# enricobolzonello/TravellingSalesmanOptimization

Measured on AMD Instinct MI355X. Metric: 2-opt delta evals/sec/node (n=4096 EUC_2D, NN(0) tour to 2-opt local optimum), higher is better.
Workload: dtype uint16 costs, int32 deltas

## Files before the change

### include/tspgpu.h

```cpp
#ifndef TSPGPU_H
#define TSPGPU_H

#ifdef __cplusplus
extern "C" {
#endif

typedef struct tspgpu_ctx tspgpu_ctx;

enum { TSPGPU_EUC_2D = 0, TSPGPU_ATT = 1, TSPGPU_CEIL_2D = 2 };

enum { TSPGPU_ELEM_AUTO = 0, TSPGPU_ELEM_F64 = 1, TSPGPU_ELEM_I32 = 2, TSPGPU_ELEM_U16 = 3 };

enum {
    TSPGPU_OPT_ELEM = 1,
    TSPGPU_OPT_KERNEL = 2,
    TSPGPU_OPT_BATCH = 3,
    TSPGPU_OPT_WGS_PER_TOUR = 4,
    TSPGPU_OPT_HISTORY = 5,
    TSPGPU_OPT_GRAPH = 6,
    TSPGPU_OPT_TIMING = 7,
    TSPGPU_OPT_BLOCK = 8,
    TSPGPU_OPT_MAX_TOURS = 9,
    TSPGPU_OPT_DEPTH = 10,
    TSPGPU_OPT_FUSED = 12,
// ... 95 lines not shown
int tspgpu_tour_copy(tspgpu_ctx *ctx, int dst, int src);
int tspgpu_tour_two_opt(tspgpu_ctx *ctx, int slot, long max_sweeps, double time_left_s, long *sweeps);
int tspgpu_tour_or_opt(tspgpu_ctx *ctx, int slot, long max_moves, double time_left_s, long *moves);
int tspgpu_tour_local_search(tspgpu_ctx *ctx, int slot, double time_left_s,
                             long *two_opt_sweeps, long *or_moves, int *rounds);
int tspgpu_tours_local_search(tspgpu_ctx *ctx, int slot0, int count, double time_left_s,
                              long *two_opt_sweeps, long *or_moves, int *rounds);
int tspgpu_time_or_sweep(tspgpu_ctx *ctx, int slot, int reps, float *ms_mean);
int tspgpu_tour_sweep_part(tspgpu_ctx *ctx, int slot, int part, int nparts, double *delta, int *a, int *b);
int tspgpu_tour_apply_move(tspgpu_ctx *ctx, int slot, int a, int b, double delta);
int tspgpu_tour_store(tspgpu_ctx *ctx, int slot, int *path, double *cost, double *last_delta);
int tspgpu_time_sweep(tspgpu_ctx *ctx, int slot, int reps, float *ms_mean);
int tspgpu_time_build(tspgpu_ctx *ctx, int reps, float *ms_mean);
int tspgpu_timing_read(tspgpu_ctx *ctx, double *sweep_ms_total, long *sweep_launches, int reset);
int tspgpu_debug_stamps(tspgpu_ctx *ctx, unsigned long long *out, int capacity_words);
int tspgpu_history(tspgpu_ctx *ctx, int *a, int *b, double *delta, int capacity, int *count);

int tspgpu_two_opt_multi_once(tspgpu_ctx *ctx, int *path, double *cost, int *nmoves,
                              int *moves_ab , double *deltas , int cap);
int tspgpu_two_opt_multi(tspgpu_ctx *ctx, int *path, double *cost, double time_left_s, long *sweeps, long *moves);
int tspgpu_tour_two_opt_multi(tspgpu_ctx *ctx, int slot, long max_sweeps, double time_left_s, long *sweeps, long *moves);
int tspgpu_time_multi_sweep(tspgpu_ctx *ctx, int slot, int reps, float *ms_mean);

int tspgpu_neighbours_build(tspgpu_ctx *ctx, int K);
int tspgpu_neighbours_get(tspgpu_ctx *ctx, int *nodes , double *weights );
int tspgpu_two_opt_nl_once(tspgpu_ctx *ctx, int *path, double *cost, int *nmoves,
                           int *moves_ab , double *deltas , int cap);
int tspgpu_two_opt_nl(tspgpu_ctx *ctx, int *path, double *cost, double time_left_s, int polish,
                      long *sweeps, long *moves, long *polish_sweeps, long *polish_moves);
int tspgpu_tour_two_opt_nl(tspgpu_ctx *ctx, int slot, long max_sweeps, double time_left_s, long *sweeps, long *moves);
// ... 49 lines not shown
```

### travellingsalesmanoptimization_amd/_lib.py

```python
import ctypes as C
import os

import numpy as np

HERE = os.path.dirname(os.path.abspath(__file__))
LIB_PATH = os.path.join(HERE, "csrc", "libtspgpu.so")

T_OK, CANCELLED, UNKNOWN, INVALID_ARGUMENT, DEADLINE_EXCEEDED = 0, 1, 2, 3, 4
RESOURCE_EXHAUSTED, FAILED_PRECONDITION, UNIMPLEMENTED, INTERNAL, UNAVAILABLE = 8, 9, 12, 13, 14

EUC_2D, ATT, CEIL_2D = 0, 1, 2
ELEM_AUTO, ELEM_F64, ELEM_I32, ELEM_U16 = 0, 1, 2, 3
OPT_ELEM, OPT_KERNEL, OPT_BATCH, OPT_WGS_PER_TOUR, OPT_HISTORY = 1, 2, 3, 4, 5
OPT_GRAPH, OPT_TIMING, OPT_BLOCK, OPT_MAX_TOURS, OPT_DEPTH, OPT_MATRIX_FREE, OPT_FUSED, OPT_SWEEP_CAP, OPT_NN_KERNEL, OPT_PIPE2 = 6, 7, 8, 9, 10, 11, 12, 13, 14, 15
OPT_PERSIST, OPT_PERSIST_EDGES, OPT_PERSIST_WINDOW, OPT_BUILD_KERNEL, OPT_STREAM_PERSIST = 16, 17, 18, 19, 20
OPT_EM_FORM = 21
OPT_OR_MATRIX_FREE = 22
INFO_OR_OTF, INFO_OR_OTF_R = 34, 35
INFO_MULTI_SWEEPS, INFO_MULTI_MOVES, INFO_MULTI_MAX_MOVES, INFO_MULTI_R, INFO_MULTI_THREADS, INFO_MULTI_NCH = 36, 37, 38, 39, 40, 41
INFO_NL_K, INFO_NL_SWEEPS, INFO_NL_MOVES, INFO_NL_POLISH_SWEEPS, INFO_NL_NODES = 42, 43, 44, 45, 46
INFO_OR_NL_SWEEPS, INFO_OR_NL_MOVES, INFO_OR_NL_MAX_MOVES, INFO_OR_NL_ROUNDS, INFO_OR_NL_STARTS = 47, 48, 49, 50, 51
INFO_NL_BATCH_TOURS, INFO_NL_BATCH_LAUNCHES, INFO_NL_BATCH_MAX_LIVE, INFO_NL_BATCH_WGS = 52, 53, 54, 55
INFO_VNS_NL_WALKS, INFO_VNS_NL_ITERATIONS, INFO_VNS_NL_ROUNDS, INFO_VNS_NL_MAX_LIVE, INFO_VNS_NL_DRY = 56, 57, 58, 59, 60
INFO_THREE_NL_W, INFO_THREE_NL_SWEEPS, INFO_THREE_NL_MOVES, INFO_THREE_NL_MAX_MOVES, INFO_THREE_NL_PHASES, INFO_THREE_NL_NODES = 62, 63, 64, 65, 66, 67
EM_FORM_AUTO, EM_FORM_RESIDENT, EM_FORM_PER_STEP = 0, 1, 2
MOPT_EXCHANGE = 1000
EXCHANGE_AUTO, EXCHANGE_HOST, EXCHANGE_RCCL = 0, 1, 2

_dp = np.ctypeslib.ndpointer(dtype=np.float64, flags="C_CONTIGUOUS")
_ip = np.ctypeslib.ndpointer(dtype=np.int32, flags="C_CONTIGUOUS")
_pd = C.POINTER(C.c_double)
_pi = C.POINTER(C.c_int)
_pl = C.POINTER(C.c_long)
_ctx = C.c_void_p

SIGNATURES = {
    "tspgpu_device_count": (C.c_int, []),
    "tspgpu_create": (C.c_int, [C.c_int, C.POINTER(_ctx)]),
    "tspgpu_destroy": (None, [_ctx]),
# ... 37 lines not shown
    "tspgpu_multi_prepare": (C.c_int, [_ctx]),
    "tspgpu_multi_set_points": (C.c_int, [_ctx, _dp, C.c_int, C.c_int]),
    "tspgpu_multi_build_costs": (C.c_int, [_ctx]),
    "tspgpu_multi_multistart_nn_2opt": (C.c_int, [_ctx, C.c_void_p, C.c_int, C.c_double, _ip, _pd, _pi, _pl]),
    "tspgpu_multi_multistart_local_search": (C.c_int, [_ctx, C.c_void_p, C.c_int, C.c_double, _ip, _pd, _pi, _pl, _pl]),
    "tspgpu_multi_nn_all": (C.c_int, [_ctx, C.c_void_p, C.c_int, C.c_double, _ip, _pd, _pi, _pi]),
    "tspgpu_tour_load": (C.c_int, [_ctx, C.c_int, _ip]),
    "tspgpu_tour_nn": (C.c_int, [_ctx, C.c_int, C.c_int]),
    "tspgpu_tour_copy": (C.c_int, [_ctx, C.c_int, C.c_int]),
    "tspgpu_tour_two_opt": (C.c_int, [_ctx, C.c_int, C.c_long, C.c_double, _pl]),
    "tspgpu_tour_store": (C.c_int, [_ctx, C.c_int, C.c_void_p, _pd, _pd]),
    "tspgpu_time_sweep": (C.c_int, [_ctx, C.c_int, C.c_int, C.POINTER(C.c_float)]),
    "tspgpu_time_build": (C.c_int, [_ctx, C.c_int, C.POINTER(C.c_float)]),
    "tspgpu_timing_read": (C.c_int, [_ctx, _pd, _pl, C.c_int]),
    "tspgpu_debug_stamps": (C.c_int, [_ctx, C.c_void_p, C.c_int]),
    "tspgpu_history": (C.c_int, [_ctx, _ip, _ip, _dp, C.c_int, _pi]),
    "tspgpu_two_opt_multi_once": (C.c_int, [_ctx, _ip, _pd, _pi, _ip, _dp, C.c_int]),
    "tspgpu_two_opt_multi": (C.c_int, [_ctx, _ip, _pd, C.c_double, _pl, _pl]),
    "tspgpu_tour_two_opt_multi": (C.c_int, [_ctx, C.c_int, C.c_long, C.c_double, _pl, _pl]),
    "tspgpu_time_multi_sweep": (C.c_int, [_ctx, C.c_int, C.c_int, C.POINTER(C.c_float)]),
    "tspgpu_neighbours_build": (C.c_int, [_ctx, C.c_int]),
    "tspgpu_neighbours_get": (C.c_int, [_ctx, _ip, C.c_void_p]),
    "tspgpu_two_opt_nl_once": (C.c_int, [_ctx, _ip, _pd, _pi, _ip, _dp, C.c_int]),
    "tspgpu_two_opt_nl": (C.c_int, [_ctx, _ip, _pd, C.c_double, C.c_int, _pl, _pl, _pl, _pl]),
    "tspgpu_tour_two_opt_nl": (C.c_int, [_ctx, C.c_int, C.c_long, C.c_double, _pl, _pl]),
    "tspgpu_time_nl_sweep": (C.c_int, [_ctx, C.c_int, C.c_int, C.POINTER(C.c_float)]),
    "tspgpu_or_opt_nl_once": (C.c_int, [_ctx, _ip, _pd, _pi, _ip, _dp, C.c_int]),
    "tspgpu_or_opt_nl": (C.c_int, [_ctx, _ip, _pd, C.c_double, _pl, _pl]),
    "tspgpu_tour_or_opt_nl": (C.c_int, [_ctx, C.c_int, C.c_long, C.c_double, _pl, _pl]),
    "tspgpu_local_search_nl": (C.c_int, [_ctx, _ip, _pd, C.c_double, _pl, _pl, _pl, _pl, _pi]),
# ... 34 lines not shown
```

### travellingsalesmanoptimization_amd/csrc/tspgpu.hip

```cpp

#include <hip/hip_runtime.h>
#include <cstddef>

#include <algorithm>
#include <chrono>
#include <cfloat>
#include <climits>
#include <cstdarg>
#include <cstdint>
#include <cstdio>
#include <cstdlib>
#include <cstring>
#include <cmath>
#include <string>
#include <type_traits>
#include <vector>

#include "tspgpu.h"
#include "tspgpu_relaunch.h"

#ifndef TSPGPU_RPC
#define TSPGPU_RPC 3
#endif

enum { E_OK = 0, E_INVALID = 3, E_DEADLINE = 4, E_EXHAUSTED = 8, E_PRECOND = 9,
       E_UNIMPL = 12, E_INTERNAL = 13, E_UNAVAILABLE = 14 };

#define TWO_OPT_EPS (-1.0E-7)

typedef unsigned long long u64;

static constexpr u64 KEY_NONE = ~0ull;
static constexpr int MAX_WGS_PER_TOUR = 1024;

// ... 2597 lines not shown
#include "tspgpu_hipmem.h"
using tspmem::Row; using tspmem::Rows;
#define MEM_GROUP __attribute__((visibility("hidden")))

struct MEM_GROUP ContextMem {
    DevBuf<int> d_flags;
    DevBuf<double2> d_pts;
    DevBuf<int2> d_ipts;
    DevBuf<double2> d_spts;
    PinBuf<int> h_ord;
    DevBuf<double> d_trace;
    HistBuf hist{nullptr, nullptr, nullptr, 0};
    DevBuf<int> hist_a, hist_b; DevBuf<double> hist_d;
    DevBuf<unsigned long long> d_stamps;
    DevBuf<u64> d_lp_slots; PinBuf<int> h_lp;
    DevBuf<int> d_lp_best;
    DevBuf<int> d_vns_rand;
    DevBuf<OrCtl> d_or;
    DevBuf<M2Ctl> d_m2;
};

struct MEM_GROUP InstanceMem {
    M2Buf m2{};
    M2Buf nlb{};
    NlbCtl *d_nlb_ctl = nullptr;
    int nlb_cap = 0;
    int *d_nlv_ord = nullptr, *d_nlv_best = nullptr;
    NlvCtl *d_nlv_ctl = nullptr;
    int nlv_cap = 0;
    DevBuf<int> d_nlv_rand; DevBuf<double> d_nlv_trace;
// ... 114 lines not shown
    int vns_mode = 0;
    long opt_lp_hello = 200000;
    int opt_lp_poll_sleep = 0;
    int opt_vns_launch_k = 65536;
    int opt_lp_fail_at = 0;
    int vns_launch_nrand = 0;
    relaunch::Gate lp_gate;
    bool lp_used = false;
    int opt_stream = 1;
    bool sp_used = false;
    int opt_sp_nch = 0;
    int opt_otf_early = 0;
    bool plan_otf_early = false;
    bool lp_shaped = false;
    int opt_lp_generic = 0;
    bool max16k = false;
    bool max8k = false;

    int opt_em_form = 0;
    int em_form = 0;
    long em_stale = 0, em_steps = 0;

    int or_batch_R = 0;
    int opt_or_otf = 0;
    int opt_or_otf_early = 0;
    int or_otf_form = 0;
    int or_otf_R = 0;

    long m2_sweeps = 0, m2_moves = 0, m2_max_k = 0;

// ... 688 lines not shown
    int e = (n + std::min(ctx->cus, 256) - 1) / std::min(ctx->cus, 256);
    if (ctx->opt_persist_edges > e) e = ctx->opt_persist_edges;
    if (e > LW_EMAX) return false;
    const int ws = (e + n / 2 + 23) & ~7;
    if (ws > n || (ws >> 3) - 1 > LW_BT) return false;
    const size_t nl = (size_t)((n + 7) & ~7);
    if ((nl >> 3) > (size_t)LW_BT) return false;
    const size_t fixed = (size_t)(e + 1) * ws * 2 + (nl + 8) * 4 + 512 + (tabu ? (nl + 16) * 2 : 0);
    int ns = 2;
    if (fixed + 2 * nl * 2 > ctx->lds_max) ns = 1;
    if (fixed + (size_t)ns * nl * 2 > ctx->lds_max) return false;
    E = e; W = (n + e - 1) / e; Ws = ws; nstage = ns; lds = fixed + (size_t)ns * nl * 2;
    return W <= ctx->cus && W <= 256;
}

static const void *lp_shaped_fn(int n, int E)
{
    if (n == 4096 && E == 16) return (const void *)k_lds2opt<true, false, false, 4096, 16>;
    if (n == 1024 && E == 4) return (const void *)k_lds2opt<true, false, false, 1024, 4>;
    return nullptr;
}

static_assert((int)relaunch::INTERNAL == (int)E_INTERNAL && (int)relaunch::GO_ON == (int)E_OK, "the driver's codes are the engine's");
static bool resident_wanted(const tspgpu_ctx *ctx) { return ctx->opt_persist == 2 || (ctx->opt_persist == 1 && ctx->opt_kernel == 0 && ctx->opt_fused == 1); }

template <typename ARGS> static int resident_args(tspgpu_ctx *ctx, ARGS &A, int slot, int W, int budget, bool first)
{
    HIP_TRY(hipMemsetAsync(ctx->d_lp_slots, 0, (size_t)2 * W * 64 + 64, ctx->stream));
    memset(&A, 0, sizeof A);
    A.S = ctx->S; A.mat = (const u16 *)ctx->d_mat.p; A.n = ctx->n; A.ld = ctx->ld; A.slot = slot; A.budget = budget;
    A.slots = ctx->d_lp_slots; A.ctl = reinterpret_cast<int *>(ctx->d_lp_slots + (size_t)2 * W * 8); A.hist = ctx->hist;
    A.hello_ticks = ctx->opt_lp_hello;
    if (ctx->opt_lp_fail_at > 0 && !first) { ctx->opt_lp_fail_at--; A.hello_ticks = -5000; }
    A.spin_ticks = 100000000;
// ... 64 lines not shown
    size_t lds = 0;
    bool win = false;
    if (ctx->opt_persist_window == 1 && persist_fits_w(ctx, E, W, lds, Ws, nstage, tabu != nullptr)) win = true;
    else if (!persist_fits(ctx, E, W, lds, tabu != nullptr)) {
        if (ctx->opt_persist_window == 2 || !persist_fits_w(ctx, E, W, lds, Ws, nstage, tabu != nullptr)) return E_OK;
        win = true;
    }
    if (ctx->lp_gate.skip_this()) return E_OK;
    HIP_TRY(ctx->d_lp_slots.reserve(((size_t)2 * LP_BT * 64 + 64) / 8));
    HIP_TRY(ctx->h_lp.reserve(16));
    if (tabu || vns) HIP_TRY(ctx->d_lp_best.reserve((size_t)ctx->ld + 16));
    const int pk = (tabu ? ctx->max8k : ctx->max16k) ? 1 : 0;
    void (*const fns[2][3][2])(PersistArgs) = {
        {{k_lds2opt<false, false>, k_lds2opt<true, false>}, {k_lds2opt<false, true>, k_lds2opt<true, true>}, {k_lds2opt<false, false, true>, k_lds2opt<true, false, true>}},
        {{k_lds2opt_w<false, false>, k_lds2opt_w<true, false>}, {k_lds2opt_w<false, true>, k_lds2opt_w<true, true>}, {k_lds2opt_w<false, false, true>, k_lds2opt_w<true, false, true>}}};
    const void *const sfn = !win && !tabu && !vns && pk && !ctx->opt_lp_generic ? lp_shaped_fn(ctx->n, E) : nullptr;
    const void *const fn = sfn ? sfn : (const void *)fns[win][tabu ? 1 : vns ? 2 : 0][pk];
    if (const int rc = ensure_max_lds(ctx, fn)) return rc;
    const double t_end = deadline_of(time_left_s);
    if (t_end >= 0 && time_left_s <= 0) { if (deadline_hit) *deadline_hit = true; *ran = true; ctx->lp_used = true; ctx->lp_window = win; ctx->lp_shaped = false; return E_OK; }
    if (vns) vns->need_rand = false;
    auto launch = [&](int budget, bool first, int &status, int &sd, auto &&fill, const double *also = nullptr) -> int {
        PersistArgs A;
        int rc = resident_args(ctx, A, slot, W, budget, first);
        A.E = E; A.nl = (ctx->n + 7) & ~7; A.Ws = Ws; A.nstage = nstage;
        if (!rc) rc = fill(A);
        return rc ? rc : launch_resident(ctx, "LDS-resident descent", fn, W, win ? LW_BT : LP_BT, lds, A, first, status, sd, also);
    };
    auto best_cost = [&]() { return reinterpret_cast<double *>(reinterpret_cast<char *>(ctx->d_tabu) + offsetof(TabuState, best_cost)); };
    auto walk_fill = [&](PersistArgs &A, double best0) -> int {
        HIP_TRY(hipMemsetAsync(ctx->d_lp_best + ctx->ld, 0, 8, ctx->stream));
        A.best0 = best0; A.best_ord = ctx->d_lp_best; A.best_dir = ctx->d_lp_best + ctx->ld; A.best_out = best_cost();
        return E_OK;
    };
    auto walk_completed = [&](int status, int sd) -> int {
        hipLaunchKernelGGL(k_lds_best_succ, dim3((ctx->n + 255) / 256), dim3(256), 0, ctx->stream, ctx->d_lp_best, ctx->d_lp_best + ctx->ld, ctx->d_best_succ, ctx->n);
        HIP_TRY(hipGetLastError());
        return descent_completed(ctx, status, sd);
    };
    relaunch::Result r;
// ... 32 lines not shown
            memcpy(&vns->best, ctx->h_lp + 8, 8);
            if (status == LP_ST_NEED_RAND) {
                vns->need_rand = vns->used + ctx->vns_launch_nrand - ctx->h_lp[5] >= vns->nrand;
                return vns->need_rand ? relaunch::STOP : relaunch::GO_ON;
            }
            if (status == LP_ST_VNS_DONE) return vns->it >= vns->k ? relaunch::STOP : relaunch::GO_ON;
            return next;
        };
        r = relaunch::drive(ctx->lp_gate, now_s, t_end, 8e-6, time_left_io,
                            [&](int budget, bool first, int &st, int &sd) { return launch(budget, first, st, sd, fill, best_cost()); }, completed, hand_over);
    } else
        r = relaunch::drive(ctx->lp_gate, now_s, t_end, 8e-6, time_left_io,
                            [&](int budget, bool first, int &st, int &sd) { return launch(budget, first, st, sd, [](PersistArgs &) -> int { return E_OK; }); },
                            [&](int status, int sd) { return descent_completed(ctx, status, sd); }, hand_over);
    if (const int rc = resident_result(ctx, r, deadline_hit, ran); rc || !*ran) return rc;
    ctx->lp_used = true; ctx->lp_window = win; ctx->lp_shaped = sfn != nullptr;
    return E_OK;
}

static bool stream_fits(const tspgpu_ctx *ctx, int &P, int &W, int &BT, int &NCH, size_t &lds)
{
    const int n = ctx->n, ld = ctx->ld;
    if (ctx->elem != TSPGPU_ELEM_U16 || ctx->otf || !ctx->symmetric || !ctx->d_mat || n < 1024 || n >= 16384) return false;
    const int cus = std::min(ctx->cus, 256);
    P = (n + cus - 1) / cus;
    W = (n + P - 1) / P;
    NCH = ld / 8 <= 1024 ? 1 : 2;
    if (ctx->opt_sp_nch > 0) NCH = ctx->opt_sp_nch;
    BT = std::max(256, ((ld / 8 + NCH - 1) / NCH + 63) & ~63);
    if (BT > 1024 || P < 2 || P > 64) return false;
    lds = sp_lds_rows(ld) + sp_lds_ord(n) + sp_lds_nodes(P) + SP_LDS_SCRATCH;
// ... 528 lines not shown
        drop_graphs(ctx);
        tspmem::reset_all(ctx->hist_a, ctx->hist_b, ctx->hist_d);
        ctx->hist = HistBuf{nullptr, nullptr, nullptr, 0}; ctx->opt_hist = 0;
        if (value > 0) {
            HIP_TRY(tspmem::alloc_all<HipMem>({{&ctx->hist_a, (size_t)value}, {&ctx->hist_b, (size_t)value}, {&ctx->hist_d, (size_t)value}}));
            ctx->hist = HistBuf{ctx->hist_a, ctx->hist_b, ctx->hist_d, (int)value};
        }
        ctx->opt_hist = (int)value;
        break;
    }
    case TSPGPU_OPT_GRAPH: ctx->opt_graph = value ? 1 : 0; break;
    case TSPGPU_OPT_TIMING: ctx->opt_timing = value ? 1 : 0; break;
    case TSPGPU_OPT_BLOCK: if (value < 0 || value > 1024) return fail(ctx, E_INVALID, "bad block"); ctx->opt_block = (int)value; ctx->plan_kernel = 0; break;
    case TSPGPU_OPT_DEPTH: if (value < 0 || value > 8) return fail(ctx, E_INVALID, "bad depth"); ctx->opt_depth = (int)value; ctx->plan_kernel = 0; break;
    case 99: ctx->opt_ablate = (int)value; drop_graphs(ctx); break;
    case 89: ctx->opt_lp_generic = value ? 1 : 0; break;
    case 90: ctx->opt_or_otf_early = value == 1 || value == 2 ? (int)value : 0; break;
    case 91: ctx->opt_otf_early = value == 1 || value == 2 ? (int)value : 0; ctx->plan_kernel = 0; drop_graphs(ctx); break;
    case 92: ctx->opt_build_tile = (int)value; break;
    case 93: ctx->opt_sp_nch = value == 1 || value == 2 ? (int)value : 0; break;
    case 94: ctx->opt_vns_launch_k = value > 0 ? (int)std::min<long>(value, 65536) : 65536; break;
    case 95: ctx->opt_lp_poll_sleep = (int)value; break;
    case 96: ctx->opt_lp_fail_at = (int)value; break;
    case 97: ctx->opt_lp_hello = value ? value : 200000; ctx->lp_gate.rearm(); break;
    case 98:
        ctx->opt_stamps = value ? 1 : 0; drop_graphs(ctx);
        if (value) HIP_TRY(ctx->d_stamps.reserve((size_t)MAX_WGS_PER_TOUR * 64));
        if (value) HIP_TRY(hipMemset(ctx->d_stamps, 0, (size_t)MAX_WGS_PER_TOUR * 64 * 8));
        break;
    case TSPGPU_OPT_MATRIX_FREE: if (value < 0 || value > 2) return fail(ctx, E_INVALID, "bad matrix-free mode"); ctx->opt_otf = (int)value; break;
// ... 82 lines not shown
    case 52: return ctx->nlb_tours;
    case 53: return ctx->nlb_launches;
    case 54: return ctx->nlb_max_live;
    case 56: return ctx->nlv_walks;
    case 57: return ctx->nlv_iterations;
    case 58: return ctx->nlv_rounds;
    case 59: return ctx->nlv_max_live;
    case 60: return ctx->nlv_dry;
    case 61: return ctx->lp_used && ctx->lp_shaped ? 1 : 0;
    case 62: return ctx->nl3_w;
    case 63: return ctx->nl3_sweeps;
    case 64: return ctx->nl3_moves;
    case 65: return ctx->nl3_max_k;
    case 66: return ctx->nl3_phases;
    case 67: return NL3_NODES;
    case 55: return ctx->have_costs && ctx->symmetric && ctx->n >= 8 ? (ctx->n + ORNL_STARTS - 1) / ORNL_STARTS : 0;
    case 12: return (ctx->built && ctx->grid_ok && ctx->opt_nn != 1 && ctx->cost_bound < 134217728.0) ? ctx->grid_G : 0;
    case 13: return ctx->grid_max_occ;
    }
    return -1;
}

int tspgpu_set_points(tspgpu_ctx *ctx, const double *xy, int n, int edge_weight_type)
{
    if (!ctx || !xy) return fail(ctx, E_INVALID, "null argument");
    if (edge_weight_type < 0 || edge_weight_type > 2) return fail(ctx, E_INVALID, "unknown edge weight type %d", edge_weight_type);
    hipSetDevice(ctx->device);
    int rc = new_instance(ctx, n);
    if (rc) return rc;
    HIP_TRY(ctx->d_pts.alloc((size_t)n));
// ... 587 lines not shown
{
    if (!ctx) return E_INVALID;
    if (sweep_ms_total) *sweep_ms_total = ctx->sweep_ms_total;
    if (sweep_launches) *sweep_launches = ctx->sweep_launches;
    if (reset) { ctx->sweep_ms_total = 0; ctx->sweep_launches = 0; }
    return E_OK;
}

int tspgpu_debug_stamps(tspgpu_ctx *ctx, unsigned long long *out, int capacity_words)
{
    if (!ctx || !out || !ctx->d_stamps) return fail(ctx, E_PRECOND, "stamps not enabled");
    hipSetDevice(ctx->device);
    HIP_TRY(hipStreamSynchronize(ctx->stream));
    const size_t words = std::min<size_t>((size_t)capacity_words, (size_t)MAX_WGS_PER_TOUR * 64);
    HIP_TRY(hipMemcpy(out, ctx->d_stamps, words * 8, hipMemcpyDeviceToHost));
    return E_OK;
}

int tspgpu_history(tspgpu_ctx *ctx, int *a, int *b, double *delta, int capacity, int *count)
{
    if (!ctx || !count) return fail(ctx, E_INVALID, "null argument");
    hipSetDevice(ctx->device);
    int ns = 0;
    if (ctx->tcap > 0) {
        HIP_TRY(hipMemcpyAsync(&ns, ctx->S.nsweeps, 4, hipMemcpyDeviceToHost, ctx->stream));
        HIP_TRY(hipStreamSynchronize(ctx->stream));
    }
    int m = std::min(std::min(ns, ctx->hist.cap), capacity);
    if (m > 0) {
        if (a) HIP_TRY(hipMemcpyAsync(a, ctx->hist.a, (size_t)m * 4, hipMemcpyDeviceToHost, ctx->stream));
// ... 1406 lines not shown
```

### travellingsalesmanoptimization_amd/csrc/tspgpu_lds2opt.inc

```
typedef unsigned v4u32 __attribute__((ext_vector_type(4)));
typedef v4u32 v4u32_a2 __attribute__((aligned(2)));
typedef short s16x2 __attribute__((ext_vector_type(2)));
typedef unsigned short u16x2 __attribute__((ext_vector_type(2)));

struct PersistArgs {
    Tours S;
    const u16 *mat;
    int n, ld, slot;
    int E;
    int nl;
    int budget;
    int Ws, nstage;
    int poll_sleep;
    u64 *slots;
    int *ctl;
    HistBuf hist;
    long hello_ticks, spin_ticks;
    unsigned long long *stamps;
    int tabu_k, tenure0, t_min, t_max, up0;
    double best0;
    int *best_ord;
    int *best_dir;
    double *trace;
    double *best_out;
    int vns_k;
    int vns_it0;
    int vns_phase;
    int vns_nrand;
    const int *vns_rand;
    int *vns_state;
};

static constexpr int LP_EMAX = 16, LP_BT = 512;
static constexpr u64 LP_KEYMASK = (1ull << 60) - 1;
static constexpr u64 LP_NONE = 0xFFFFFFFFFull << 24;
static constexpr int LP_DBIAS = 131072;

__device__ __forceinline__ void lp_ld128(const u64 *p, u64 &a, u64 &b)
{
    v4u32 r;
    asm volatile("global_load_dwordx4 %0, %1, off sc1\n\ts_waitcnt vmcnt(0)" : "=v"(r) : "v"(p) : "memory");
    a = r.x | (u64)r.y << 32; b = r.z | (u64)r.w << 32;
}
__device__ __forceinline__ void lp_st128(u64 *p, u64 a, u64 b)
{
// ... 14 lines not shown
#undef STEP
    return __builtin_amdgcn_readlane(x, 63);
}
__device__ __forceinline__ unsigned lp_pk_add(unsigned a, unsigned b)
{
    return __builtin_bit_cast(unsigned, (u16x2)(__builtin_bit_cast(u16x2, a) + __builtin_bit_cast(u16x2, b)));
}
__device__ __forceinline__ unsigned lp_pk_sub(unsigned a, unsigned b)
{
    return __builtin_bit_cast(unsigned, (s16x2)(__builtin_bit_cast(s16x2, a) - __builtin_bit_cast(s16x2, b)));
}
__device__ __forceinline__ unsigned lp_pk_min(unsigned a, unsigned b)
{
    return __builtin_bit_cast(unsigned, __builtin_elementwise_min(__builtin_bit_cast(s16x2, a), __builtin_bit_cast(s16x2, b)));
}
template <bool PK16, bool TABU, bool VNS = false, int NLC = 0, int EC = 0>
__global__ void __launch_bounds__(LP_BT) k_lds2opt(PersistArgs A)
{
    extern __shared__ __attribute__((aligned(16))) unsigned char smem[];
    constexpr int EMAX = LP_EMAX, BT = LP_BT;
    constexpr bool SH = NLC > 0;
    constexpr int WC = NLC / (EC > 0 ? EC : 1);
    typedef __attribute__((address_space(4))) const PersistArgs c_PersistArgs;
    static_assert(!SH || (PK16 && !TABU && !VNS), "the shaped form is the plain packed descent");
    static_assert(!SH || ((NLC & (NLC - 1)) == 0 && NLC % 16 == 0 && NLC / 8 <= LP_BT), "shaped n: a power of two, at most 8 cells a thread");
    static_assert(!SH || (EC >= 2 && EC % 2 == 0 && EC <= LP_EMAX && NLC % EC == 0 && NLC / EC <= 256), "shaped E: even, W = n / E <= 256");
    constexpr unsigned POISON = PK16 ? 16383u : 65535u;
    const int n = SH ? NLC : A.n, nl = SH ? NLC : A.nl, ld = A.ld, E = SH ? EC : A.E, W = SH ? WC : (int)gridDim.x,
              wg = (int)blockIdx.x, tid = (int)threadIdx.x, t = A.slot;
#define LP_WRAP_HI(p) if constexpr (SH) p &= NLC - 1; else if (p >= n) p -= n
#define LP_WRAP_LO(p) if constexpr (SH) p &= NLC - 1; else if (p < 0) p += n
#define LP_WRAP_EQS(p) if constexpr (SH) p &= NLC - 1; else if (p == n) p = 0
#define LP_TID (SH ? tid_sweep : tid)
#define LP_LM0 (SH ? lm0_sweep : lm0)
#define LP_WRAP_EQ(p) (SH ? ((p) & (NLC - 1)) : ((p) == n ? 0 : (p)))
    const size_t tn = (size_t)t * n;
    u16 *rows = reinterpret_cast<u16 *>(smem);
    u16 *wt16 = reinterpret_cast<u16 *>(smem + (size_t)(E + 1) * nl * 2);
    unsigned *wt = reinterpret_cast<unsigned *>(wt16);
// ... 84 lines not shown
        const unsigned ownlab = wt16[2 * oc + 1];
        unsigned offs[8];
        if (act) {
            const v4u32 la = *reinterpret_cast<const v4u32 *>(wt + m0), lb = *reinterpret_cast<const v4u32 *>(wt + m0 + 4);
            offs[0] = la.x >> 16 << 1; offs[1] = la.y >> 16 << 1; offs[2] = la.z >> 16 << 1; offs[3] = la.w >> 16 << 1;
            offs[4] = lb.x >> 16 << 1; offs[5] = lb.y >> 16 << 1; offs[6] = lb.z >> 16 << 1; offs[7] = lb.w >> 16 << 1;
        }
        v4u32 R[EMAX + 1];
#pragma unroll
        for (int r = 0; r <= EMAX; r++) {
            if ((need >> r) & 1) {
                const int x = __builtin_amdgcn_readlane((int)ownlab, r);
                if (act) R[r] = *reinterpret_cast<const v4u32 *>(A.mat + (size_t)x * ld + m0);
            }
        }
        if constexpr (SH) asm volatile("" : "+s"(need));
        const int last = 31 - __builtin_clz(need);
        int left = __builtin_popcount(need);
        unsigned char *bufT = reinterpret_cast<unsigned char *>(rows + (size_t)last * nl);
        unsigned char *bufS = reinterpret_cast<unsigned char *>(stage);
        unsigned char *bprev = nullptr;
        int rprev = 0;
        auto gather = [&](const unsigned char *buf, int rdst) __attribute__((always_inline)) {
            if (act) {
                unsigned g[8];
#pragma unroll
                for (int v = 0; v < 8; v++) g[v] = *reinterpret_cast<const u16 *>(buf + offs[v]);
                const v4u32 out = {g[0] | g[1] << 16, g[2] | g[3] << 16, g[4] | g[5] << 16, g[6] | g[7] << 16};
                *reinterpret_cast<v4u32 *>(rows + (size_t)rdst * nl + m0) = out;
            }
        };
// ... 23 lines not shown
        gather(bprev, rprev);
        __syncthreads();
        if constexpr (TABU) {
            if (tid <= E && ((need >> tid) & 1)) {
                int p = k0 + tid; if (p >= n) p -= n;
                int pl = p - 1; if (pl < 0) pl += n;
                int pr = p + 1; if (pr == n) pr = 0;
                rows[(size_t)tid * nl + pl] = (u16)POISON; rows[(size_t)tid * nl + pr] = (u16)POISON;
                if (n < nl && (pl == 0 || pr == 0)) rows[(size_t)tid * nl + n] = (u16)POISON;
            }
            __syncthreads();
        }
    };
    const unsigned allrows = (2u << E) - 1u;
    reload(allrows);

    int status = LP_ST_RUNNING;
    if (cap >= 0 && kd >= cap) status = LP_ST_CAPPED;
    int tenure = A.tenure0, tup = A.up0, iters = 0;
    double best = A.best0;
    if (TABU && A.tabu_k <= 0) status = LP_ST_CAPPED;
    int vit = A.vns_it0, vcur = 0;
    u16 *vns_lab = rows;
    auto vns_mirror = [&]() __attribute__((always_inline)) { if (n < nl && tid == 0) wt[n] = wt[0]; };
#include "tspgpu_lds_vns.inc"
    if constexpr (VNS) {
        if (A.vns_phase == 1 && status == LP_ST_RUNNING) {
            const int st = vns_step(false);
            if (st != LP_ST_RUNNING) status = st;
        }
// ... 238 lines not shown
                    const int v = __builtin_ctz(cms);
                    cms &= cms - 1;
                    const int m = m0s + v, mp = LP_WRAP_EQ(m + 1);
                    if (lane < rcnts) {
                        const int r = rlos + lane, k = k0 + r;
                        const unsigned xa = rows[(size_t)r * nl + m], yb = rows[(size_t)(r + 1) * nl + mp];
                        const int d = (int)xa + (int)yb - (int)wt16[2 * k] - (int)wt16[2 * m];
                        bool ok = d == dmin;
                        if constexpr (TABU) ok = ok && xa != POISON && !((etmask >> r) & 1);
                        if (ok) offer(k, m, xa, yb);
                    }
                }
            }
            if (mykey != ~0ull) __hip_atomic_fetch_min(&scr[0], mykey, __ATOMIC_RELAXED, __HIP_MEMORY_SCOPE_WORKGROUP);
        }
        __syncthreads();
        const u64 kmin = scr[0];
        const bool have = found ? mykey == kmin : LP_TID == 0;
        LP_PHASE(1);
        sdone++;
        exchange(sdone, have, found ? mykey : LP_NONE, mypay, r0, r1, A.spin_ticks);
        if (r0 == 0) { give_up(LP_ST_LOST); return; }
        LP_PHASE(2);
        kd++;
        const bool nomove = (r0 >> 24) == 0xFFFFFFFFFull;
        if (nomove && !TABU) {
            lastd = 0;
            if (wg == 0 && LP_TID == 0 && t == 0 && kd <= A.hist.cap) { A.hist.a[kd - 1] = -1; A.hist.b[kd - 1] = -1; A.hist.d[kd - 1] = 0.0; }
            if constexpr (!VNS) { status = LP_ST_OPTIMUM; break; }
            else {
// ... 165 lines not shown
                int r = cell - k0; if (r < 0) r += n;
                if (r <= E && !((need >> r) & 1)) {
                    rows[(size_t)r * nl + back] = (u16)val;
                    rows[(size_t)r * nl + won] = (u16)POISON;
                }
            }
            __syncthreads();
        }
        if (n < nl) {
            if (tid < nrow) rows[(size_t)tid * nl + n] = rows[(size_t)tid * nl];
            if (tid == nrow) wt[n] = wt[0];
            if (TABU && tid == nrow + 1) age16[n] = age16[0];
            __syncthreads();
        }
        LP_PHASE(3);
        if (need) { reload(need); nreload++; nrows += __builtin_popcount(need); }
        LP_PHASE(4);
        if (clk && wg == 0 && sdone < 4000) A.stamps[8192 + sdone] = ((unsigned long long)M << 48) | (wall_clock64() & 0xFFFFFFFFFFFFull);
        }
        if constexpr (TABU) {
            iters++;
            const double cur = cost0 + (double)sumd;
            if (!nomove && cur < best) {
                best = cur;
                if (tid < E) A.best_ord[k0 + tid] = (int)wt16[2 * (k0 + tid) + 1];
                if (wg == 0 && tid == 0) { A.best_dir[0] = dir; A.best_dir[1] = 1; }
            }
            if (wg == 0 && tid == 0) A.trace[iters - 1] = cur;
            for (int q = tid; q < nl; q += BT) { const unsigned a = age16[q]; if (a != 0xFFFFu) age16[q] = (u16)(a + 1); }
            if (tenure == A.t_max || tenure == A.t_min) tup = !tup;
            tenure += tup ? 1 : -1;
            if (iters >= A.tabu_k) status = LP_ST_CAPPED;
// ... 29 lines not shown
        S_.pos[tn_ + lab] = p;                                                                                            \
        S_.succ[tn_ + lab] = dir > 0 ? (int)wt16[2 * pn + 1] : (int)wt16[2 * pp + 1];                                     \
        reinterpret_cast<int *>(S_.dnb + tn_)[lab] = dir > 0 ? (int)wt16[2 * p] : (int)wt16[2 * pp];                      \
    }                                                                                                                     \
    if (wg == 0 && tid == 0) {                                                                                            \
        S_.dir[t_] = dir;                                                                                                 \
        S_.cost[t_] = cost0 + (double)sumd;                                                                               \
        S_.nsweeps[t_] = kd;                                                                                              \
        if (sdone > 0) S_.last_delta[t_] = (double)lastd;                                                                 \
        if (status == LP_ST_OPTIMUM || status == LP_ST_CAPPED) S_.done[t_] = 1;                                           \
        if constexpr (TABU || VNS) *A.best_out = best;                                                                    \
        if constexpr (VNS) { A.vns_state[0] = vit; A.vns_state[1] = vcur; A.vns_state[2] = status == LP_ST_NEED_RAND ? 1 : 0; } \
        ctl_[1] = status; ctl_[2] = sdone;                                                                                \
    }
    if constexpr (SH) {
        static_assert(std::is_same_v<decltype(&k_lds2opt<PK16, TABU, VNS, NLC, EC>), void (*)(PersistArgs)>, "PersistArgs must stay the kernel's only argument");
        c_PersistArgs *Ak = (c_PersistArgs *)__builtin_amdgcn_kernarg_segment_ptr();
        asm volatile("" : "+s"(Ak));
        const int tk = Ak->slot;
        const size_t tnk = (size_t)tk * n;
        LP_WRITE_BACK(Ak->S, tk, tnk, Ak->ctl)
    } else {
        LP_WRITE_BACK(A.S, t, tn, A.ctl)
    }
#undef LP_WRITE_BACK
}

__global__ void __launch_bounds__(256) k_lds_best_succ(const int *__restrict__ best_ord, const int *__restrict__ best_dir, int *__restrict__ best_succ, int n)
{
    if (!best_dir[1]) return;
    const int p = blockIdx.x * 256 + threadIdx.x;
// ... 5 lines not shown
```

### travellingsalesmanoptimization_amd/engine.py

```python
import ctypes as C

import numpy as np

from . import _lib
from ._lib import (DEADLINE_EXCEEDED, ELEM_AUTO, ELEM_F64, ELEM_I32, EUC_2D, T_OK)


class TspGpuError(RuntimeError):
    def __init__(self, code, msg):
        super().__init__(f"tspgpu error {code}: {msg}")
        self.code = code


class Engine:
    def __init__(self, device=0):
        self.L = _lib.load()
        self.ctx = C.c_void_p()
        rc = self.L.tspgpu_create(device, C.byref(self.ctx))
        if rc != T_OK:
            raise TspGpuError(rc, "tspgpu_create failed (no gfx950 device visible?)")
        self.n = 0

    def close(self):
        if self.ctx:
# ... 14 lines not shown
    def set_option(self, opt, value):
        self._ck(self.L.tspgpu_set_option(self.ctx, opt, int(value)))

    def info(self):
        names = ["n", "ld", "elem", "kernel", "wgs_per_tour", "lds_bytes", "block", "symmetric", "cus", "depth", "matrix_free", "fused",
                 "nn_grid", "nn_grid_max_cell", "pipe2", "persist", "persist_wgs", "persist_edges", "persist_lds", "persist_window_cells",
                 "persist_window", "persist_handed", "persist_sweeps", "vns_mode", "stream_persist",
                 "otf_kernel", "ceil_int", "em_form", "em_stale", "em_steps", "or_batch_r", "or_single_r",
                 "or_block", "or_nch", "or_otf", "or_otf_R",
                 "multi_sweeps", "multi_moves", "multi_max_moves", "multi_r", "multi_block", "multi_nch",
                 "nl_k", "nl_sweeps", "nl_moves", "nl_polish_sweeps", "nl_nodes",
                 "or_nl_sweeps", "or_nl_moves", "or_nl_max_moves", "or_nl_rounds", "or_nl_starts",
                 "nl_batch_tours", "nl_batch_launches", "nl_batch_max_live", "nl_batch_wgs",
                 "vns_nl_walks", "vns_nl_iterations", "vns_nl_rounds", "vns_nl_max_live", "vns_nl_dry",
                 "persist_shaped",
                 "three_nl_w", "three_nl_sweeps", "three_nl_moves", "three_nl_max_moves", "three_nl_phases", "three_nl_nodes"]
        return {k: int(self.L.tspgpu_info(self.ctx, i)) for i, k in enumerate(names)}

    def set_points(self, xy, kind=EUC_2D):
        xy = np.ascontiguousarray(xy, dtype=np.float64).reshape(-1)
        self.n = len(xy) // 2
        self._ck(self.L.tspgpu_set_points(self.ctx, xy, self.n, kind))

    def build_costs(self, fetch=False):
        if fetch:
            out = np.empty((self.n, self.n), dtype=np.float64)
            self._ck(self.L.tspgpu_build_costs(self.ctx, out.ctypes.data))
            return out
        self._ck(self.L.tspgpu_build_costs(self.ctx, None))
        return None

# ... 489 lines not shown
```

Baseline: 1192 billion.

## Keep a tour-ordered global copy of cost rows for shaped LDS 2-opt reloads

Adds an n×n u16 global buffer that mirrors the LDS-resident rows in tour order. After each 2-opt move the changed segment is written back, and reloads fetch contiguous 16-byte chunks from this copy, mirrored where the segment was reversed, instead of gathering through the permutation from the original matrix. The aim is to cut the cost of the row-reload gather in the persistent descent kernel. In exchange it adds write-back traffic, an extra n² buffer, and vmcnt waits before the move reduction, and it only applies to the shaped n=4096/1024 kernels.

```diff
diff --git a/include/tspgpu.h b/include/tspgpu.h
--- a/include/tspgpu.h
+++ b/include/tspgpu.h
@@ -133,6 +133,7 @@
 int tspgpu_time_build(tspgpu_ctx *ctx, int reps, float *ms_mean);
 int tspgpu_timing_read(tspgpu_ctx *ctx, double *sweep_ms_total, long *sweep_launches, int reset);
 int tspgpu_debug_stamps(tspgpu_ctx *ctx, unsigned long long *out, int capacity_words);
+int tspgpu_debug_tmat(tspgpu_ctx *ctx, unsigned short *out, size_t cells);
 int tspgpu_history(tspgpu_ctx *ctx, int *a, int *b, double *delta, int capacity, int *count);
 
 int tspgpu_two_opt_multi_once(tspgpu_ctx *ctx, int *path, double *cost, int *nmoves,
diff --git a/travellingsalesmanoptimization_amd/_lib.py b/travellingsalesmanoptimization_amd/_lib.py
--- a/travellingsalesmanoptimization_amd/_lib.py
+++ b/travellingsalesmanoptimization_amd/_lib.py
@@ -23,6 +23,7 @@
 INFO_NL_BATCH_TOURS, INFO_NL_BATCH_LAUNCHES, INFO_NL_BATCH_MAX_LIVE, INFO_NL_BATCH_WGS = 52, 53, 54, 55
 INFO_VNS_NL_WALKS, INFO_VNS_NL_ITERATIONS, INFO_VNS_NL_ROUNDS, INFO_VNS_NL_MAX_LIVE, INFO_VNS_NL_DRY = 56, 57, 58, 59, 60
 INFO_THREE_NL_W, INFO_THREE_NL_SWEEPS, INFO_THREE_NL_MOVES, INFO_THREE_NL_MAX_MOVES, INFO_THREE_NL_PHASES, INFO_THREE_NL_NODES = 62, 63, 64, 65, 66, 67
+INFO_PERSIST_TMAT = 68
 EM_FORM_AUTO, EM_FORM_RESIDENT, EM_FORM_PER_STEP = 0, 1, 2
 MOPT_EXCHANGE = 1000
 EXCHANGE_AUTO, EXCHANGE_HOST, EXCHANGE_RCCL = 0, 1, 2
@@ -90,6 +91,7 @@
     "tspgpu_time_build": (C.c_int, [_ctx, C.c_int, C.POINTER(C.c_float)]),
     "tspgpu_timing_read": (C.c_int, [_ctx, _pd, _pl, C.c_int]),
     "tspgpu_debug_stamps": (C.c_int, [_ctx, C.c_void_p, C.c_int]),
+    "tspgpu_debug_tmat": (C.c_int, [_ctx, C.c_void_p, C.c_size_t]),
     "tspgpu_history": (C.c_int, [_ctx, _ip, _ip, _dp, C.c_int, _pi]),
     "tspgpu_two_opt_multi_once": (C.c_int, [_ctx, _ip, _pd, _pi, _ip, _dp, C.c_int]),
     "tspgpu_two_opt_multi": (C.c_int, [_ctx, _ip, _pd, C.c_double, _pl, _pl]),
diff --git a/travellingsalesmanoptimization_amd/csrc/tspgpu.hip b/travellingsalesmanoptimization_amd/csrc/tspgpu.hip
--- a/travellingsalesmanoptimization_amd/csrc/tspgpu.hip
+++ b/travellingsalesmanoptimization_amd/csrc/tspgpu.hip
@@ -18,6 +18,7 @@
 
 #include "tspgpu.h"
 #include "tspgpu_relaunch.h"
+#include "tspgpu_lds_tmat.h"
 
 #ifndef TSPGPU_RPC
 #define TSPGPU_RPC 3
@@ -2645,6 +2646,7 @@
     DevBuf<int> hist_a, hist_b; DevBuf<double> hist_d;
     DevBuf<unsigned long long> d_stamps;
     DevBuf<u64> d_lp_slots; PinBuf<int> h_lp;
+    DevBuf<u16> d_lp_tmat;
     DevBuf<int> d_lp_best;
     DevBuf<int> d_vns_rand;
     DevBuf<OrCtl> d_or;
@@ -2789,6 +2791,8 @@
     bool plan_otf_early = false;
     bool lp_shaped = false;
     int opt_lp_generic = 0;
+    bool lp_tmat = false;
+    int opt_lp_no_tmat = 0;
     bool max16k = false;
     bool max8k = false;
 
@@ -3507,10 +3511,10 @@
     return W <= ctx->cus && W <= 256;
 }
 
-static const void *lp_shaped_fn(int n, int E)
-{
-    if (n == 4096 && E == 16) return (const void *)k_lds2opt<true, false, false, 4096, 16>;
-    if (n == 1024 && E == 4) return (const void *)k_lds2opt<true, false, false, 1024, 4>;
+static const void *lp_shaped_fn(int n, int E, bool tmat)
+{
+    if (n == 4096 && E == 16) return tmat ? (const void *)k_lds2opt<true, false, false, 4096, 16, true> : (const void *)k_lds2opt<true, false, false, 4096, 16>;
+    if (n == 1024 && E == 4) return tmat ? (const void *)k_lds2opt<true, false, false, 1024, 4, true> : (const void *)k_lds2opt<true, false, false, 1024, 4>;
     return nullptr;
 }
 
@@ -3605,16 +3609,19 @@
     void (*const fns[2][3][2])(PersistArgs) = {
         {{k_lds2opt<false, false>, k_lds2opt<true, false>}, {k_lds2opt<false, true>, k_lds2opt<true, true>}, {k_lds2opt<false, false, true>, k_lds2opt<true, false, true>}},
         {{k_lds2opt_w<false, false>, k_lds2opt_w<true, false>}, {k_lds2opt_w<false, true>, k_lds2opt_w<true, true>}, {k_lds2opt_w<false, false, true>, k_lds2opt_w<true, false, true>}}};
-    const void *const sfn = !win && !tabu && !vns && pk && !ctx->opt_lp_generic ? lp_shaped_fn(ctx->n, E) : nullptr;
+    const bool shaped = !win && !tabu && !vns && pk && !ctx->opt_lp_generic && lp_shaped_fn(ctx->n, E, false);
+    bool tm = shaped && !ctx->opt_lp_no_tmat;
+    if (tm && ctx->d_lp_tmat.reserve((size_t)ctx->n * ctx->n) != hipSuccess) { (void)hipGetLastError(); tm = false; }
+    const void *const sfn = shaped ? lp_shaped_fn(ctx->n, E, tm) : nullptr;
     const void *const fn = sfn ? sfn : (const void *)fns[win][tabu ? 1 : vns ? 2 : 0][pk];
     if (const int rc = ensure_max_lds(ctx, fn)) return rc;
     const double t_end = deadline_of(time_left_s);
-    if (t_end >= 0 && time_left_s <= 0) { if (deadline_hit) *deadline_hit = true; *ran = true; ctx->lp_used = true; ctx->lp_window = win; ctx->lp_shaped = false; return E_OK; }
+    if (t_end >= 0 && time_left_s <= 0) { if (deadline_hit) *deadline_hit = true; *ran = true; ctx->lp_used = true; ctx->lp_window = win; ctx->lp_shaped = false; ctx->lp_tmat = false; return E_OK; }
     if (vns) vns->need_rand = false;
     auto launch = [&](int budget, bool first, int &status, int &sd, auto &&fill, const double *also = nullptr) -> int {
         PersistArgs A;
         int rc = resident_args(ctx, A, slot, W, budget, first);
-        A.E = E; A.nl = (ctx->n + 7) & ~7; A.Ws = Ws; A.nstage = nstage;
+        A.E = E; A.nl = (ctx->n + 7) & ~7; A.Ws = Ws; A.nstage = nstage; A.tmat = tm ? ctx->d_lp_tmat.p : nullptr;
         if (!rc) rc = fill(A);
         return rc ? rc : launch_resident(ctx, "LDS-resident descent", fn, W, win ? LW_BT : LP_BT, lds, A, first, status, sd, also);
     };
@@ -3677,7 +3684,7 @@
                             [&](int budget, bool first, int &st, int &sd) { return launch(budget, first, st, sd, [](PersistArgs &) -> int { return E_OK; }); },
                             [&](int status, int sd) { return descent_completed(ctx, status, sd); }, hand_over);
     if (const int rc = resident_result(ctx, r, deadline_hit, ran); rc || !*ran) return rc;
-    ctx->lp_used = true; ctx->lp_window = win; ctx->lp_shaped = sfn != nullptr;
+    ctx->lp_used = true; ctx->lp_window = win; ctx->lp_shaped = sfn != nullptr; ctx->lp_tmat = tm;
     return E_OK;
 }
 
@@ -4236,6 +4243,7 @@
     case TSPGPU_OPT_BLOCK: if (value < 0 || value > 1024) return fail(ctx, E_INVALID, "bad block"); ctx->opt_block = (int)value; ctx->plan_kernel = 0; break;
     case TSPGPU_OPT_DEPTH: if (value < 0 || value > 8) return fail(ctx, E_INVALID, "bad depth"); ctx->opt_depth = (int)value; ctx->plan_kernel = 0; break;
     case 99: ctx->opt_ablate = (int)value; drop_graphs(ctx); break;
+    case 88: ctx->opt_lp_no_tmat = value ? 1 : 0; break;
     case 89: ctx->opt_lp_generic = value ? 1 : 0; break;
     case 90: ctx->opt_or_otf_early = value == 1 || value == 2 ? (int)value : 0; break;
     case 91: ctx->opt_otf_early = value == 1 || value == 2 ? (int)value : 0; ctx->plan_kernel = 0; drop_graphs(ctx); break;
@@ -4348,6 +4356,7 @@
     case 65: return ctx->nl3_max_k;
     case 66: return ctx->nl3_phases;
     case 67: return NL3_NODES;
+    case 68: return ctx->lp_used && ctx->lp_shaped && ctx->lp_tmat ? 1 : 0;
     case 55: return ctx->have_costs && ctx->symmetric && ctx->n >= 8 ? (ctx->n + ORNL_STARTS - 1) / ORNL_STARTS : 0;
     case 12: return (ctx->built && ctx->grid_ok && ctx->opt_nn != 1 && ctx->cost_bound < 134217728.0) ? ctx->grid_G : 0;
     case 13: return ctx->grid_max_occ;
@@ -4965,6 +4974,16 @@
     HIP_TRY(hipStreamSynchronize(ctx->stream));
     const size_t words = std::min<size_t>((size_t)capacity_words, (size_t)MAX_WGS_PER_TOUR * 64);
     HIP_TRY(hipMemcpy(out, ctx->d_stamps, words * 8, hipMemcpyDeviceToHost));
+    return E_OK;
+}
+
+int tspgpu_debug_tmat(tspgpu_ctx *ctx, unsigned short *out, size_t cells)
+{
+    if (!ctx || !out) return fail(ctx, E_INVALID, "null argument");
+    if (!ctx->d_lp_tmat) return fail(ctx, E_PRECOND, "no tour-ordered copy was kept");
+    hipSetDevice(ctx->device);
+    HIP_TRY(hipStreamSynchronize(ctx->stream));
+    HIP_TRY(hipMemcpy(out, ctx->d_lp_tmat, std::min(cells, ctx->d_lp_tmat.n) * sizeof(u16), hipMemcpyDeviceToHost));
     return E_OK;
 }
 
diff --git a/travellingsalesmanoptimization_amd/csrc/tspgpu_lds2opt.inc b/travellingsalesmanoptimization_amd/csrc/tspgpu_lds2opt.inc
--- a/travellingsalesmanoptimization_amd/csrc/tspgpu_lds2opt.inc
+++ b/travellingsalesmanoptimization_amd/csrc/tspgpu_lds2opt.inc
@@ -29,6 +29,7 @@
     int vns_nrand;
     const int *vns_rand;
     int *vns_state;
+    u16 *tmat;
 };
 
 static constexpr int LP_EMAX = 16, LP_BT = 512;
@@ -73,7 +74,7 @@
 {
     return __builtin_bit_cast(unsigned, __builtin_elementwise_min(__builtin_bit_cast(s16x2, a), __builtin_bit_cast(s16x2, b)));
 }
-template <bool PK16, bool TABU, bool VNS = false, int NLC = 0, int EC = 0>
+template <bool PK16, bool TABU, bool VNS = false, int NLC = 0, int EC = 0, bool TM = false>
 __global__ void __launch_bounds__(LP_BT) k_lds2opt(PersistArgs A)
 {
     extern __shared__ __attribute__((aligned(16))) unsigned char smem[];
@@ -82,6 +83,7 @@
     constexpr int WC = NLC / (EC > 0 ? EC : 1);
     typedef __attribute__((address_space(4))) const PersistArgs c_PersistArgs;
     static_assert(!SH || (PK16 && !TABU && !VNS), "the shaped form is the plain packed descent");
+    static_assert(!TM || SH, "the tour-ordered copy needs the shaped form: n == nl a power of two, k0 = wg * E, no overlapping workgroup");
     static_assert(!SH || ((NLC & (NLC - 1)) == 0 && NLC % 16 == 0 && NLC / 8 <= LP_BT), "shaped n: a power of two, at most 8 cells a thread");
     static_assert(!SH || (EC >= 2 && EC % 2 == 0 && EC <= LP_EMAX && NLC % EC == 0 && NLC / EC <= 256), "shaped E: even, W = n / E <= 256");
     constexpr unsigned POISON = PK16 ? 16383u : 65535u;
@@ -196,7 +198,7 @@
                 if (act) R[r] = *reinterpret_cast<const v4u32 *>(A.mat + (size_t)x * ld + m0);
             }
         }
-        if constexpr (SH) asm volatile("" : "+s"(need));
+        if constexpr (SH && !TM) asm volatile("" : "+s"(need));
         const int last = 31 - __builtin_clz(need);
         int left = __builtin_popcount(need);
         unsigned char *bufT = reinterpret_cast<unsigned char *>(rows + (size_t)last * nl);
@@ -250,6 +252,101 @@
     };
     const unsigned allrows = (2u << E) - 1u;
     reload(allrows);
+    auto tm_rsrc = [&]() __attribute__((always_inline)) {
+        c_PersistArgs *Ak = (c_PersistArgs *)__builtin_amdgcn_kernarg_segment_ptr();
+        asm volatile("" : "+s"(Ak));
+        return __builtin_amdgcn_make_buffer_rsrc(Ak->tmat, 0, NLC * NLC * 2, 0x00020000);
+    };
+    constexpr int TM_SC1 = 16;
+    if constexpr (TM) {
+        const auto rs = tm_rsrc();
+#pragma unroll 4
+        for (int i = tid; i < EC * (NLC / 8); i += BT) {
+            const int row = i / (NLC / 8), c = i & (NLC / 8 - 1);
+            const unsigned x = wt16[2 * (k0 + row) + 1];
+            const v4u32 v = *reinterpret_cast<const v4u32 *>(rows + (size_t)row * NLC + 8 * c);
+            __builtin_amdgcn_raw_buffer_store_b128(v, rs, (int)((x * NLC + 8 * c) * 2), 0, TM_SC1);
+        }
+    }
+    auto fetch_tm = [&](unsigned need, int lo, int M, int tidv) __attribute__((always_inline)) {
+        if constexpr (!TM) return;
+        const auto rs = tm_rsrc();
+        const int lane = tid & 63;
+        const unsigned ownlab = wt16[2 * ((k0 + min(lane, EC)) & (NLC - 1)) + 1];
+        int start = 0;
+        const int cls = act ? lds_tmat::chunk_class(m0, lo, M, NLC, start) : (int)lds_tmat::CELLWISE;
+        v4u32 R[EC > 0 ? EC : 1], Rc = {0, 0, 0, 0};
+#pragma unroll
+        for (int r = 0; r < EC; r++)
+            if ((need >> r) & 1)
+                R[r] = __builtin_amdgcn_raw_buffer_load_b128(rs, start * 2, __builtin_amdgcn_readlane((int)ownlab, r) * (NLC * 2), TM_SC1);
+        asm volatile("" : "+s"(need));
+        const bool copy = (need >> EC) & 1;
+        const unsigned xc = (unsigned)__builtin_amdgcn_readlane((int)ownlab, EC);
+        if (copy && act) {
+            c_PersistArgs *Ak = (c_PersistArgs *)__builtin_amdgcn_kernarg_segment_ptr();
+            asm volatile("" : "+s"(Ak));
+            Rc = *reinterpret_cast<const v4u32 *>(Ak->mat + (size_t)(xc * (unsigned)Ak->ld) + m0);
+        }
+        int cw[3];
+        lds_tmat::cellwise_chunks(lo, M, NLC, cw);
+        const int sr = tidv / 24, si = tidv - sr * 24;
+        const bool sact = sr < EC && ((need >> sr) & 1);
+        const int sq = (si < 8 ? cw[0] : si < 16 ? cw[1] : cw[2]) * 8 + (si & 7);
+        const unsigned sx = wt16[2 * (k0 + min(sr, EC - 1)) + 1];
+        const u16 sv = __builtin_amdgcn_raw_buffer_load_b16(rs, (int)((sx * NLC + lds_tmat::src_cell(sq, lo, M, NLC)) * 2), 0, TM_SC1);
+#pragma unroll
+        for (int r = 0; r < EC; r++) {
+            if ((need >> r) & 1) {
+                const v4u32 v = R[r];
+                const v4u32 m = {__builtin_amdgcn_alignbit(v.w, v.w, 16), __builtin_amdgcn_alignbit(v.z, v.z, 16),
+                                 __builtin_amdgcn_alignbit(v.y, v.y, 16), __builtin_amdgcn_alignbit(v.x, v.x, 16)};
+                if (cls != lds_tmat::CELLWISE) *reinterpret_cast<v4u32 *>(rows + (size_t)r * NLC + m0) = cls == lds_tmat::MIRROR ? m : v;
+            }
+        }
+        if (sact) rows[(size_t)sr * NLC + sq] = sv;
+        asm volatile("" :: "v"((unsigned)sv));
+        if (copy) {
+            if (act) {
+                v4u32 v = Rc;
+                if ((int)(xc >> 3) == tid) {
+                    const unsigned sel = (xc & 7u) >> 1;
+                    unsigned c[4] = {v.x, v.y, v.z, v.w};
+#pragma unroll
+                    for (int q = 0; q < 4; q++)
+                        if ((unsigned)q == sel) c[q] = (xc & 1u) ? (c[q] & 0xffffu) | (POISON << 16) : (c[q] & 0xffff0000u) | POISON;
+                    v = v4u32{c[0], c[1], c[2], c[3]};
+                }
+                *reinterpret_cast<v4u32 *>(stage + m0) = v;
+            }
+            __syncthreads();
+            if (act) {
+                const v4u32 la = *reinterpret_cast<const v4u32 *>(wt + m0), lb = *reinterpret_cast<const v4u32 *>(wt + m0 + 4);
+                const unsigned l[8] = {la.x >> 16, la.y >> 16, la.z >> 16, la.w >> 16, lb.x >> 16, lb.y >> 16, lb.z >> 16, lb.w >> 16};
+                unsigned g[8];
+#pragma unroll
+                for (int v = 0; v < 8; v++) g[v] = stage[l[v]];
+                const v4u32 out = {g[0] | g[1] << 16, g[2] | g[3] << 16, g[4] | g[5] << 16, g[6] | g[7] << 16};
+                *reinterpret_cast<v4u32 *>(rows + (size_t)EC * NLC + m0) = out;
+            }
+        }
+        __syncthreads();
+    };
+    auto write_back_tm = [&](int lo, int M, int tidv) __attribute__((always_inline)) {
+        if constexpr (!TM) return;
+        const auto rs = tm_rsrc();
+        const int nch = lds_tmat::wb_count(lo, M), c0 = lds_tmat::wb_first(lo);
+        const int lg = nch > 1 ? 32 - __builtin_clz(nch - 1) : 0;
+        const int j = tidv & ((1 << lg) - 1), rpi = BT >> lg;
+        if (j < nch) {
+            const int c = (c0 + j) & (NLC / 8 - 1);
+            for (int row = tidv >> lg; row < EC; row += rpi) {
+                const unsigned x = wt16[2 * (k0 + row) + 1];
+                const v4u32 v = *reinterpret_cast<const v4u32 *>(rows + (size_t)row * NLC + 8 * c);
+                __builtin_amdgcn_raw_buffer_store_b128(v, rs, (int)((x * NLC + 8 * c) * 2), 0, TM_SC1);
+            }
+        }
+    };
 
     int status = LP_ST_RUNNING;
     if (cap >= 0 && kd >= cap) status = LP_ST_CAPPED;
@@ -518,6 +615,7 @@
             }
             if (mykey != ~0ull) __hip_atomic_fetch_min(&scr[0], mykey, __ATOMIC_RELAXED, __HIP_MEMORY_SCOPE_WORKGROUP);
         }
+        if constexpr (TM) asm volatile("s_waitcnt vmcnt(0)" ::: "memory");
         __syncthreads();
         const u64 kmin = scr[0];
         const bool have = found ? mykey == kmin : LP_TID == 0;
@@ -713,8 +811,12 @@
             __syncthreads();
         }
         LP_PHASE(3);
-        if (need) { reload(need); nreload++; nrows += __builtin_popcount(need); }
+        if (need) {
+            if constexpr (TM) fetch_tm(need, lo, M, LP_TID); else reload(need);
+            nreload++; nrows += __builtin_popcount(need);
+        }
         LP_PHASE(4);
+        if constexpr (TM) { write_back_tm(lo, M, LP_TID); LP_PHASE2(3); }
         if (clk && wg == 0 && sdone < 4000) A.stamps[8192 + sdone] = ((unsigned long long)M << 48) | (wall_clock64() & 0xFFFFFFFFFFFFull);
         }
         if constexpr (TABU) {
@@ -774,7 +876,7 @@
         ctl_[1] = status; ctl_[2] = sdone;                                                                                \
     }
     if constexpr (SH) {
-        static_assert(std::is_same_v<decltype(&k_lds2opt<PK16, TABU, VNS, NLC, EC>), void (*)(PersistArgs)>, "PersistArgs must stay the kernel's only argument");
+        static_assert(std::is_same_v<decltype(&k_lds2opt<PK16, TABU, VNS, NLC, EC, TM>), void (*)(PersistArgs)>, "PersistArgs must stay the kernel's only argument");
         c_PersistArgs *Ak = (c_PersistArgs *)__builtin_amdgcn_kernarg_segment_ptr();
         asm volatile("" : "+s"(Ak));
         const int tk = Ak->slot;
diff --git a/travellingsalesmanoptimization_amd/csrc/tspgpu_lds_tmat.h b/travellingsalesmanoptimization_amd/csrc/tspgpu_lds_tmat.h
--- /dev/null
+++ b/travellingsalesmanoptimization_amd/csrc/tspgpu_lds_tmat.h
@@ -0,0 +1,38 @@
+#pragma once
+
+#if defined(__HIPCC__) || defined(__CUDACC__)
+#define TMAT_HD __host__ __device__
+#else
+#define TMAT_HD
+#endif
+
+namespace lds_tmat {
+
+TMAT_HD inline bool in_range(int q, int lo, int M, int n) { return ((q - lo) & (n - 1)) < M; }
+
+TMAT_HD inline int src_cell(int q, int lo, int M, int n) { return in_range(q, lo, M, n) ? (2 * lo + M - 1 - q) & (n - 1) : q; }
+
+enum { SAME = 0, MIRROR = 1, CELLWISE = 2 };
+TMAT_HD inline int chunk_class(int q0, int lo, int M, int n, int &start)
+{
+    const int d0 = (q0 - lo) & (n - 1);
+    start = q0;
+    if (d0 >= M && d0 + 7 < n) return SAME;
+    if (d0 + 7 < M) {
+        const int a = (2 * lo + M - 1 - (q0 + 7)) & (n - 1);
+        if (a + 8 <= n) { start = a; return MIRROR; }
+    }
+    return CELLWISE;
+}
+
+TMAT_HD inline void cellwise_chunks(int lo, int M, int n, int c[3])
+{
+    c[0] = lo >> 3;
+    c[1] = ((lo + M) & (n - 1)) >> 3;
+    c[2] = ((2 * lo + M - 1) & (n - 1)) >> 3;
+}
+
+TMAT_HD inline int wb_first(int lo) { return lo >> 3; }
+TMAT_HD inline int wb_count(int lo, int M) { return ((lo & 7) + M + 7) >> 3; }
+
+}
diff --git a/travellingsalesmanoptimization_amd/engine.py b/travellingsalesmanoptimization_amd/engine.py
--- a/travellingsalesmanoptimization_amd/engine.py
+++ b/travellingsalesmanoptimization_amd/engine.py
@@ -52,7 +52,8 @@
                  "nl_batch_tours", "nl_batch_launches", "nl_batch_max_live", "nl_batch_wgs",
                  "vns_nl_walks", "vns_nl_iterations", "vns_nl_rounds", "vns_nl_max_live", "vns_nl_dry",
                  "persist_shaped",
-                 "three_nl_w", "three_nl_sweeps", "three_nl_moves", "three_nl_max_moves", "three_nl_phases", "three_nl_nodes"]
+                 "three_nl_w", "three_nl_sweeps", "three_nl_moves", "three_nl_max_moves", "three_nl_phases", "three_nl_nodes",
+                 "persist_tmat"]
         return {k: int(self.L.tspgpu_info(self.ctx, i)) for i, k in enumerate(names)}
 
     def set_points(self, xy, kind=EUC_2D):
```

New measurement: 1380 billion, median of 6. +15.8%, better.
